# cjpurackal/nice-slam-cpp

Measured on AMD Instinct MI355X. Metric: mapping rays/sec (and ms/iter) on CoFusion room1 at 1/2/4/8 MI355X, higher is better.
Workload: dtype f32

## Files before the change

include/nsk.h:

```cpp
#ifndef NSK_H
#define NSK_H

#include <stddef.h>
#include <stdint.h>

#ifdef __cplusplus
extern "C" {
#endif

#define NSK_COARSE 0
#define NSK_MIDDLE 1
#define NSK_FINE 2
#define NSK_COLOR 3

#define NSK_GRAD_GRIDS 1u
#define NSK_GRAD_DECODERS 2u
#define NSK_GRAD_RAYS 4u

#define NSK_GROUP_DECODERS 0
#define NSK_GROUP_COARSE 1
#define NSK_GROUP_MIDDLE 2
#define NSK_GROUP_FINE 3
#define NSK_GROUP_COLOR 4
#define NSK_GROUP_CAMERA 5
// ... 13 lines not shown
int nsk_set_matmul_mode(nsk_ctx* ctx, int mode);
int nsk_set_backward_mode(nsk_ctx* ctx, int mode);

int nsk_set_sort_mode(nsk_ctx* ctx, int mode);
int nsk_set_tuning(nsk_ctx* ctx, const char* key, int value);

int nsk_set_bound(nsk_ctx* ctx, const float h_bound[6]);

int nsk_set_render_opts(nsk_ctx* ctx, int n_samples, int n_surface, int lindisp, float perturb, int occupancy,
                        uint64_t seed);

int nsk_grid_upload(nsk_ctx* ctx, int level, const float* h_czyx, int C, int Z, int Y, int X);
int nsk_grid_download(nsk_ctx* ctx, int level, float* h_czyx);
int nsk_grid_grad_download(nsk_ctx* ctx, int level, float* h_czyx);
int nsk_set_mask(nsk_ctx* ctx, int level, const uint8_t* h_mask_zyx);

int nsk_frustum_mask(nsk_ctx* ctx, int level, const float* d_depth, int H, int W, float fx, float fy, float cx, float cy,
                     const float h_c2w[16], uint8_t* h_mask_out);

int nsk_keyframe_overlap(nsk_ctx* ctx, int N, const float* d_rays_o, const float* d_rays_d, const float* d_gt_depth, int n_samples,
                         int H, int W, float fx, float fy, float cx, float cy, int K, const float* h_c2w, float* h_percent);

size_t nsk_decoder_param_count(int which);
int nsk_decoder_upload(nsk_ctx* ctx, int which, const float* h_packed, size_t n);
int nsk_decoder_download(nsk_ctx* ctx, int which, float* h_packed, size_t n);
int nsk_decoder_grad_download(nsk_ctx* ctx, int which, float* h_packed, size_t n);
int nsk_decoder_set_trainable(nsk_ctx* ctx, int which, int trainable);

int nsk_render_forward(nsk_ctx* ctx, int stage, int N, const float* d_rays_o, const float* d_rays_d,
                       const float* d_gt_depth, float gt_depth_max, float* d_rgb, float* d_depth, float* d_var,
// ... 101 lines not shown
```

nice-slam-cpp_amd/csrc/nsk.hip:

```cpp
#include "../../include/nsk.h"
#include "nsk_device.h"
#include "nsk_train.h"
#include "nsk_bf16.h"
#include "nsk_mesh.h"
#include "nsk_buf.h"

#include <dlfcn.h>
#include <cstdarg>
#include <algorithm>
#include <cmath>
#include <cstdio>
#include <cstring>
#include <memory>
#include <string>
#include <vector>

#define NSK_VERSION 100

static thread_local std::string g_err;
static int fail(const char* fmt, ...)
{
    char buf[512];
    va_list ap; va_start(ap, fmt); vsnprintf(buf, sizeof(buf), fmt, ap); va_end(ap);
    g_err = buf;
// ... 106 lines not shown
        const int v = v0 + threadIdx.x;
        const bool on = v < nvox && mask[v];
        const unsigned long long b = __builtin_amdgcn_ballot_w64(on);
        if (lane == 0) wsum[wave] = __builtin_popcountll(b);
        __syncthreads();
        int off = base;
        for (int w = 0; w < wave; ++w) off += wsum[w];
        if (on) idx[off + __builtin_popcountll(b & ((1ull << lane) - 1ull))] = v;
        __syncthreads();
        if (threadIdx.x == 0) { int t = 0; for (int w = 0; w < 16; ++w) t += wsum[w]; base += t; }
        __syncthreads();
    }
    if (threadIdx.x == 0) *count = base;
}

struct XSeg { const int* idx; int n4; float* slab; float* buf; int blk_end;
              const float* slabs; int nslabs, slab_stride; };
struct XArgs { XSeg s[10]; int n; int gather; };
__global__ __launch_bounds__(256) void k_xchg_multi(XArgs A)
{
    int r = 0;
    while (r < A.n - 1 && (int)blockIdx.x >= A.s[r].blk_end) ++r;
    const XSeg& S = A.s[r];
    const int b0 = r ? A.s[r - 1].blk_end : 0;
    if (S.slabs) {
        __shared__ f4 red[32][8];
        const int pi = threadIdx.x & 7, sg = threadIdx.x >> 3;
        const int i = (blockIdx.x - b0) * 8 + pi;
        f4 part = (f4)(0.f);
        if (i < S.n4) {
// ... 478 lines not shown
__global__ void k_gather_pixels(int n, const int* __restrict__ pi, const int* __restrict__ pj, int W, const float* __restrict__ depth,
                                const float* __restrict__ color, float* __restrict__ gd, float* __restrict__ gc)
{
    const int r = blockIdx.x * blockDim.x + threadIdx.x;
    if (r >= n) return;
    const size_t p = (size_t)pj[r] * W + pi[r];
    gd[r] = depth[p];
    if (color && gc) { gc[3 * r] = color[3 * p]; gc[3 * r + 1] = color[3 * p + 1]; gc[3 * r + 2] = color[3 * p + 2]; }
}

struct HipAlloc {
    static int alloc(void** p, size_t bytes) { return (int)hipMalloc(p, bytes); }
    static void free(void* p) { (void)hipFree(p); }
};
template <typename T> using Buf = DevBuf<T, HipAlloc>;

struct GridState {
    int C = 0, Z = 0, Y = 0, X = 0;
    size_t n = 0;
    Buf<float> v, m, s;
    Buf<uint8_t> mask;
    size_t g_off = 0;
    Buf<int> midx; int nmask = 0; bool midx_dirty = true;
};
struct DecState {
    int n = 0;
    Buf<float> p, m, s;
    Buf<float> fimg, bimg;
    Buf<int> fidx, bidx;
    Buf<int> finv, binv;
    Buf<int> inv16;
    Buf<int> invh;
    Buf<float> bimg16; Buf<int> bidx16; int bfrag16_n = 0; bool bimg16_dirty = true;
    Buf<float> fimg16; Buf<int> fidx16; int frag16_n = 0, fimg16_f = 0, tail_off = 0, tail16_off = 0, np16 = 3, cq16 = 2;
    int fimg_n = 0, bimg_n = 0;
    int trainable = 0;
// ... 39 lines not shown
    int cap_rollback[NSK_NUM_GROUPS] = {0, 0, 0, 0, 0, 0};
    int ws_flip = 0;
    struct GraphRec { bool stale = false; int flip = 0; hipGraph_t graph = nullptr; hipGraphExec_t exec = nullptr; hipGraphNode_t adam_node = nullptr; bool has_adam = false; CapAdam adam; std::vector<CapVec> vecs; };
    std::vector<GraphRec> graphs;
    bool touched[NSK_NUM_GROUPS] = {false, false, false, false, false, false};
    bool deterministic = false;
    bool roctx = false;
    int tune_fwd_occ_cost = 0, tune_no_occ_role = 0;
    int tune_fwd_fine_cost = 0, tune_fwd_color_cost = 0;
    bool median_fused_pending = false;
    int tune_no_deferred_median = 0;
    int tune_no_fused_median = 0;
    int tune_frozen_cost = 0;
    int tune_frozen_cost_rays = 0;
    int tune_frozen_mid_pct = 100;
    int tune_no_frozen_kernel = 0;
    const uint8_t* ray_mask = nullptr;
    struct DMax { const float* gt = nullptr; const uint8_t* keep = nullptr; int n = 0; } dmax;
    float* xextra = nullptr; size_t xextra_n = 0;
    int sort_mode = -1;
    bool sorted = false;
    struct Prep { bool valid = false; int stage = 0, N = 0, S = 0; const float* ro = nullptr; const float* rd = nullptr; const float* gt = nullptr;
                  float gtmax = 0.f; const uint8_t* mask = nullptr; bool sorted = false; int done = 0; RParams R; DMax dmax; } prep, req;
    int tune_no_piggyback = 0;
    int pend_w = -1, pend_nb = 0;
    int dbg_M = 0, dbg_S = 0;
    int bwd_mode = 2;
    int matmul_mode = 2;
    double last_bytes = 0, last_flops = 0; int last_samples = 0;
    struct Mesh {
// ... 125 lines not shown
    HIPCHK(hipGetDeviceProperties(&prop, device));
    if (strncmp(prop.gcnArchName, "gfx950", 6) != 0) return fail("nsk_ctx_create: device arch %s, this library is built for gfx950 only", prop.gcnArchName);
    std::unique_ptr<nsk_ctx> owner(new nsk_ctx());
    nsk_ctx* c = owner.get();
    c->device = device;
    c->num_cu = prop.multiProcessorCount;
    if (hip_stream) { c->stream = (hipStream_t)hip_stream; c->own_stream = false; }
    else { HIPCHK(hipStreamCreateWithFlags(&c->stream, hipStreamNonBlocking)); c->own_stream = true; }
    const float b[6] = {-4.5f, 3.82f, -1.5f, 2.02f, -3.0f, 2.76f};
    memcpy(c->R.bound, b, sizeof(b));
    c->R.n_samples = 32; c->R.n_surface = 16; c->R.lindisp = 0; c->R.occupancy = 0; c->R.perturb = 0.f; c->R.seed = 0;
    CHK(dev_alloc(c->d_bound, 6, "the bound"));
    HIPCHK(hipMemcpy(c->d_bound, b, sizeof(b), hipMemcpyHostToDevice));
    CHK(dev_alloc(c->scal, 16, "the scalars"));
    HIPCHK(hipMemset(c->scal, 0, 16 * sizeof(float)));
    CHK(set_lds(k_decode_fwd<0>, fwd_img_floats(0) * 4)); CHK(set_lds(k_decode_fwd<1>, fwd_img_floats(1) * 4));
    CHK(set_lds(k_decode_fwd<2>, fwd_img_floats(2) * 4)); CHK(set_lds(k_decode_fwd<3>, fwd_img_floats(3) * 4));
#define SETB(W) \
    CHK(set_lds(k_decode_bwd<W, false>, bwd_lds_bytes(W, false))); CHK(set_lds(k_decode_bwd<W, true>, bwd_lds_bytes(W, false))); \
    CHK(set_lds(k_decode_bwd_train<W, false>, bwd_lds_bytes(W, true))); CHK(set_lds(k_decode_bwd_train<W, true>, bwd_lds_bytes(W, true)));
    SETB(0) SETB(1) SETB(2) SETB(3)
#undef SETB
    CHK(set_lds(k_median_thr, 16384 * 4));
    CHK(set_lds(k_decode_fwd_multi, 160 * 1024)); CHK(set_lds(k_decode_fwd_multi_bf16<8>, 160 * 1024)); CHK(set_lds(k_decode_fwd_multi_bf16<8, 2>, 160 * 1024)); CHK(set_lds(k_decode_fwd_multi_occ<8>, 160 * 1024));
    CHK(set_lds(k_decode_bwd_multi<false>, 160 * 1024 - 256)); CHK(set_lds(k_decode_bwd_multi<true>, 160 * 1024));
    CHK(set_lds(k_decode_bwd_frozen<false>, 160 * 1024 - 256));
    CHK(set_lds(k_decode_bwd_track, 160 * 1024)); CHK(set_lds(k_decode_bwd_multi_full<false>, 160 * 1024)); CHK(set_lds(k_decode_bwd_multi_full<true>, 160 * 1024));
    CHK(set_lds(k_decode_fwd_dump<0>, 160 * 1024)); CHK(set_lds(k_decode_fwd_dump<1>, 160 * 1024)); CHK(set_lds(k_decode_fwd_dump<2>, 160 * 1024));
    *out = owner.release();
    return 0;
// ... 40 lines not shown

extern "C" int nsk_set_backward_mode(nsk_ctx* c, int mode)
{
    if (!c) return fail("null ctx");
    if (mode != 0 && mode != 2) return fail("nsk_set_backward_mode: 0 (fp32 MFMA chains) or 2 (two fp16 pieces, default)");
    c->bwd_mode = mode;
    return 0;
}

extern "C" int nsk_set_tuning(nsk_ctx* c, const char* key, int value)
{
    if (!c || !key) return fail("nsk_set_tuning: null argument");
    if (!strcmp(key, "frozen_cost")) { c->tune_frozen_cost = value; return 0; }
    if (!strcmp(key, "frozen_cost_rays")) { c->tune_frozen_cost_rays = value; return 0; }
    if (!strcmp(key, "no_frozen_kernel")) { c->tune_no_frozen_kernel = value; return 0; }
    if (!strcmp(key, "no_piggyback")) { c->tune_no_piggyback = value; return 0; }
    if (!strcmp(key, "frozen_mid_pct")) { if (value < 10 || value > 1000) return fail("nsk_set_tuning: frozen_mid_pct out of range"); c->tune_frozen_mid_pct = value; return 0; }
    if (!strcmp(key, "no_fused_median")) { c->tune_no_fused_median = value; return 0; }
    if (!strcmp(key, "no_deferred_median")) { c->tune_no_deferred_median = value; return 0; }
    if (!strcmp(key, "fwd_fine_cost")) { c->tune_fwd_fine_cost = value; return 0; }
    if (!strcmp(key, "fwd_occ_cost")) { c->tune_fwd_occ_cost = value; return 0; }
    if (!strcmp(key, "no_occ_role")) { c->tune_no_occ_role = value; return 0; }
    if (!strcmp(key, "fwd_color_cost")) { c->tune_fwd_color_cost = value; return 0; }
    if (!strcmp(key, "deterministic")) { c->deterministic = value != 0; return 0; }
    if (!strcmp(key, "roctx")) { c->roctx = value != 0; return 0; }
    if (!strcmp(key, "lattice_slab")) { if (value < 0 || value >= (1 << 26)) return fail("nsk_set_tuning: lattice_slab must be 0 (automatic) or a node count below 2^26"); c->mesh.slab = value; return 0; }
    return fail("nsk_set_tuning: unknown key '%s'", key);
}

extern "C" int nsk_set_ray_mask(nsk_ctx* c, const uint8_t* d_keep)
// ... 43 lines not shown
        c->slab_n = n;
    }
    HIPCHK(hipMemsetAsync(c->slab, 0, n * sizeof(float), c->stream));
    return 0;
}

static int grid_upload(nsk_ctx* c, GridState& G, const float* h, int C, int Z, int Y, int X)
{
    size_t nvox = (size_t)Z * Y * X, n = nvox * 32;
    bool realloc_ = n != G.n;
    if (realloc_) {
        CHK(grow_begin(c, GROW_STALE_GRAPHS));
        G = GridState();
        CHK(dev_alloc(G.v, n, "a grid level")); CHK(dev_alloc(G.m, n, "a grid level's first moment")); CHK(dev_alloc(G.s, n, "a grid level's second moment"));
    }
    if (G.Z != Z || G.Y != Y || G.X != X) { if (G.mask) { CHK(grow_begin(c, GROW_STALE_GRAPHS)); G.mask.reset(); } }
    G.C = C; G.Z = Z; G.Y = Y; G.X = X; G.n = n; G.midx_dirty = true;
    std::vector<float> t(n);
    for (int ch = 0; ch < 32; ++ch)
        for (size_t v = 0; v < nvox; ++v) t[v * 32 + ch] = h[(size_t)ch * nvox + v];
    HIPCHK(hipMemcpyAsync(G.v, t.data(), n * 4, hipMemcpyHostToDevice, c->stream));
    HIPCHK(hipMemsetAsync(G.m, 0, n * 4, c->stream));
    HIPCHK(hipMemsetAsync(G.s, 0, n * 4, c->stream));
    HIPCHK(hipStreamSynchronize(c->stream));
    if (realloc_) CHK(rebuild_slab(c));
    return 0;
}
extern "C" int nsk_grid_upload(nsk_ctx* c, int level, const float* h, int C, int Z, int Y, int X)
{
    if (!c || !h) return fail("nsk_grid_upload: null argument");
    if (!which_ok(level)) return fail("nsk_grid_upload: bad level %d", level);
// ... 28 lines not shown
extern "C" int nsk_grid_grad_download(nsk_ctx* c, int level, float* h)
{
    if (!c || !h || !which_ok(level)) return fail("nsk_grid_grad_download: bad argument");
    CHK(grid_fetch(c, level, c->slab + c->grid[level].g_off, h));
    GridState& G = c->grid[level];
    if (G.mask) {
        const size_t nvox = G.n / 32;
        std::vector<uint8_t> m(nvox);
        HIPCHK(hipMemcpy(m.data(), G.mask, nvox, hipMemcpyDeviceToHost));
        for (int ch = 0; ch < 32; ++ch)
            for (size_t v = 0; v < nvox; ++v) if (!m[v]) h[(size_t)ch * nvox + v] = 0.f;
    }
    return 0;
}

extern "C" int nsk_set_mask(nsk_ctx* c, int level, const uint8_t* h_mask)
{
    if (!c || !which_ok(level)) return fail("nsk_set_mask: bad argument");
    GridState& G = c->grid[level];
    if (!G.n) return fail("nsk_set_mask: grid level %d not uploaded", level);
    if (c->capturing) return fail("nsk_set_mask: not while a graph is being captured");
    HIPCHK(hipStreamSynchronize(c->stream));
    size_t nvox = G.n / 32;
    G.midx_dirty = true;
    invalidate_graphs(c);
    if (c->slab) HIPCHK(hipMemsetAsync(c->slab + G.g_off, 0, G.n * 4, c->stream));
    if (!h_mask) { G.mask.reset(); return 0; }
    if (!G.mask) CHK(dev_alloc(G.mask, nvox, "the voxel mask"));
    HIPCHK(hipMemcpy(G.mask, h_mask, nvox, hipMemcpyHostToDevice));
    return 0;
}

static void seg_fwd(std::vector<int>& idx, int quad0, int KQ, int Wofs, int ld, int col0, int kvalid)
{
    for (int rt = 0; rt < 2; ++rt) for (int q = 0; q < KQ; ++q) for (int lane = 0; lane < 64; ++lane) for (int i = 0; i < 4; ++i) {
        int o = 16 * rt + (lane & 15), k = 16 * q + 4 * (lane >> 4) + i;
        idx[((size_t)(quad0 + rt * KQ + q) * 64 + lane) * 4 + i] = k < kvalid ? Wofs + o * ld + col0 + k : -1;
    }
}
static void seg_bwd(std::vector<int>& idx, int quad0, int RT, int Wofs, int ld, int col0, int rvalid)
{
    const int KQ = 2;
    for (int rt = 0; rt < RT; ++rt) for (int q = 0; q < KQ; ++q) for (int lane = 0; lane < 64; ++lane) for (int i = 0; i < 4; ++i) {
        int r = 16 * rt + (lane & 15), k = 16 * q + 4 * (lane >> 4) + i;
// ... 884 lines not shown
    }
    return T.ntri[case_index];
}

static int flush_pending(nsk_ctx* c)
{
    if (c->pend_w < 0) return 0;
    const int w = c->pend_w, np = c->dec[w].n, n4 = (np + 3) & ~3;
    ProfScope ps(c, "dec_grad_reduce");
    k_dec_grad_reduce<<<dim3((np + 255) / 256, 8), 256, 0, c->stream>>>(np, n4, c->pend_nb, c->ws.dec_slabs, c->slab + c->dec[w].g_off);
    HIPCHK(hipGetLastError());
    c->pend_w = -1;
    return 0;
}

static int backward_core(nsk_ctx* c, int stage, int N, int S, const float* ro, const float* rd, unsigned flags, float* g_ro, float* g_rd,
                         float* d_loss = nullptr, const float* dyn_resid = nullptr)
{
    const bool rays = (flags & NSK_GRAD_RAYS) != 0;
    const bool grids = (flags & NSK_GRAD_GRIDS) != 0;
    const int M = N * S;
    CHK(flush_pending(c));
    MultiArgs MA;
    memset(&MA, 0, sizeof(MA));
    int n = 0, cost[3], train_role = -1; size_t lds = 0;
    for (int q = 2; q >= 0; --q) {
        int w = STAGE_DEC[stage][q];
        if (w < 0) continue;
        bool train = (flags & NSK_GRAD_DECODERS) && c->dec[w].trainable;
        if (!train && !grids && !rays) continue;
// ... 2 lines not shown
        A.grid = grid_dev(c, w, grids);
        A.masks = c->ws.masks[w];
        A.g_raw = c->ws.g_raw;
        A.g_rays_o = g_ro; A.g_rays_d = g_rd;
        A.dyn_resid = dyn_resid; A.dyn_n = N;
        A.g_dec = train ? c->ws.dec_slabs : c->slab + c->dec[w].g_off;
        A.flags = flags & 0xffu;
        if (w != 0 && (!train || w != 2)) CHK(ensure_bimg16(c, w));
        if (train && w != 2) {
            if (c->ws.hsave_M[w] != M) return fail("backward of trainable decoder %d: its forward must run with the decoder already trainable (block outputs not saved)", w);
            A.hsave = c->ws.hsave[w];
        }
        MA.which[n] = w; MA.train[n] = train ? 1 : 0;
        const int frozen_cost = rays ? (c->tune_frozen_cost_rays > 0 ? c->tune_frozen_cost_rays : 330) : (c->tune_frozen_cost > 0 ? c->tune_frozen_cost : 205);
        cost[n] = train ? 1000 : (w == 1 ? frozen_cost * c->tune_frozen_mid_pct / 100 : frozen_cost);
        lds = std::max(lds, bwd_lds_bytes(w, train));
        if (train) train_role = (train_role == -1 && w != 2) ? n : -2;
        if (train) c->touched[NSK_GROUP_DECODERS] = true;
        if (grids) c->touched[NSK_GROUP_COARSE + w] = true;
        ++n;
    }
    if (dyn_resid && (train_role != -1 || !rays || c->deterministic || c->bwd_mode == 0 || n == 0 || N > NSK_MEDIAN_FUSED_MAX))
        return fail("backward_core: the deferred median mask needs the Tracker's launch (frozen decoders, ray gradients)");
    const int separate = c->deterministic ? 1 : 0;
    if ((n == 0 || train_role == -2 || separate) && d_loss) { ProfScope ps(c, "loss_sum"); k_sum<<<1, 1024, 0, c->stream>>>(N, c->ws.ray_loss, d_loss); }
    if (n == 0) return 0;
    if (train_role == -2 || separate) {
        for (int r = 0; r < n; ++r)
            CHK(launch_decode_bwd(c, MA.which[r], M, S, ro, rd, MA.train[r] != 0, rays, flags, g_ro, g_rd));
        return 0;
// ... 285 lines not shown
extern "C" int nsk_frustum_mask(nsk_ctx* c, int level, const float* d_depth, int H, int W, float fx, float fy, float cx, float cy,
                                const float h_c2w[16], uint8_t* h_mask_out)
{
    if (!c || !which_ok(level) || !d_depth || !h_c2w) return fail("nsk_frustum_mask: bad argument");
    GridState& G = c->grid[level];
    if (!G.n) return fail("nsk_frustum_mask: grid level %d not uploaded", level);
    HIPCHK(hipSetDevice(c->device));
    const size_t nvox = G.n / 32;
    G.midx_dirty = true;
    if (c->capturing) return fail("nsk_frustum_mask: not while a graph is being captured");
    bool live = false;
    for (auto& R : c->graphs) live = live || !R.stale;
    if (live) { HIPCHK(hipStreamSynchronize(c->stream)); invalidate_graphs(c); }
    if (c->slab) HIPCHK(hipMemsetAsync(c->slab + G.g_off, 0, G.n * 4, c->stream));
    CHK(grow(c, G.mask, nvox, "the voxel mask", 0));
    if (level == NSK_COARSE) {
        HIPCHK(hipMemsetAsync(G.mask, 1, nvox, c->stream));
    } else {
        CHK(grow(c, c->fr_tmp, nvox * 9 + 16, "the frustum scratch", 0));
        float* dep = reinterpret_cast<float*>(c->fr_tmp.get()); float* zz = dep + nvox;
        uint8_t* inimg = reinterpret_cast<uint8_t*>(zz + nvox);
        unsigned int* dmax = reinterpret_cast<unsigned int*>(c->scal + 4);
        FrustumArgs A;
        memcpy(A.bound, c->R.bound, sizeof(A.bound));
        invert4(h_c2w, A.w2c);
        A.cam[0] = h_c2w[3]; A.cam[1] = h_c2w[7]; A.cam[2] = h_c2w[11];
        A.Z = G.Z; A.Y = G.Y; A.X = G.X; A.H = H; A.W = W; A.fx = fx; A.fy = fy; A.cx = cx; A.cy = cy;
        HIPCHK(hipMemsetAsync(dmax, 0, 4, c->stream));
        int blocks = (int)((nvox + 255) / 256);
        k_frustum_pass1<<<blocks, 256, 0, c->stream>>>(A, d_depth, dep, zz, inimg, dmax);
        k_frustum_pass2<<<blocks, 256, 0, c->stream>>>(A, dep, zz, inimg, dmax, G.mask);
        HIPCHK(hipGetLastError());
    }
    if (h_mask_out) {
        HIPCHK(hipMemcpyAsync(h_mask_out, G.mask, nvox, hipMemcpyDeviceToHost, c->stream));
        HIPCHK(hipStreamSynchronize(c->stream));
    }
    return 0;
}

extern "C" int nsk_keyframe_overlap(nsk_ctx* c, int N, const float* d_ro, const float* d_rd, const float* d_gt_depth, int n_samples,
                                    int H, int W, float fx, float fy, float cx, float cy, int K, const float* h_c2w, float* h_percent)
{
    if (!c || !d_ro || !d_rd || !d_gt_depth || !h_c2w || !h_percent) return fail("nsk_keyframe_overlap: null argument");
    if (N <= 0 || n_samples <= 0 || K < 0) return fail("nsk_keyframe_overlap: bad sizes");
    if (K == 0) return 0;
    HIPCHK(hipSetDevice(c->device));
    std::vector<float> w2c((size_t)K * 16);
// ... 537 lines not shown
```

nice-slam-cpp_amd/csrc/nsk_device.h:

```cpp
#pragma once
#include <hip/hip_runtime.h>
#include <stdint.h>
#include "nsk_layout.h"

typedef float f4 __attribute__((ext_vector_type(4)));

struct RParams {
    float bound[6];
    int n_samples, n_surface, lindisp, occupancy;
    float perturb;
    unsigned long long seed;
};

struct GridD {
    const float* v;
    float* g;
    const uint8_t* mask;
    int Z, Y, X;
};

#define NSK_INF __builtin_huge_valf()

__device__ __forceinline__ f4 mfma4(float a, float b, f4 c) { return __builtin_amdgcn_mfma_f32_16x16x4f32(a, b, c, 0, 0, 0); }
__device__ __forceinline__ void lds_fence() { asm volatile("s_waitcnt lgkmcnt(0)" ::: "memory"); }
// ... 667 lines not shown
    const f4* img;
    const void* img16;
    const f4* bimg;
    const void* bimg16;
    int img_f4;
    float* out;
    unsigned long long* masks;
    f4* hsave;
    const float* g_raw;
    float* g_rays_o; float* g_rays_d;
    float* g_dec;
    unsigned flags;
    float* dump;
    const float* dyn_resid;
    int dyn_n;
};

template <typename T>
__device__ __forceinline__ T ld32(const void* base, unsigned byte_off) { return *reinterpret_cast<const T*>(reinterpret_cast<const char*>(base) + byte_off); }
__device__ __forceinline__ int ray_of(const DecArgs& A, int mm) { return A.S_magic ? (int)__umulhi((unsigned)mm, A.S_magic) : mm; }
struct __attribute__((packed, aligned(4))) Ray3 { float x, y, z; };
__device__ __forceinline__ void sample_point(const DecArgs& A, int mm, float& px, float& py, float& pz, float& zz, int& n)
{
    if (A.pts) { px = A.pts[3 * mm]; py = A.pts[3 * mm + 1]; pz = A.pts[3 * mm + 2]; zz = 0.f; n = 0; return; }
    n = ray_of(A, mm);
    zz = A.z[mm];
    const Ray3 o = *reinterpret_cast<const Ray3*>(A.rays_o + 3 * n), d = *reinterpret_cast<const Ray3*>(A.rays_d + 3 * n);
    px = add_rn(o.x, mul_rn(d.x, zz));
    py = add_rn(o.y, mul_rn(d.y, zz));
    pz = add_rn(o.z, mul_rn(d.z, zz));
// ... 485 lines not shown
template <int K> struct ImgRegs { f4 v[K]; };
template <int NT, int K>
__device__ __forceinline__ void image_issue(ImgRegs<K>& R, const f4* __restrict__ src, int n4)
{
#pragma unroll
    for (int u = 0; u < K; ++u) { const int i = u * NT + (int)threadIdx.x; R.v[u] = i < n4 ? src[i] : (f4)(0.f); }
}
template <int NT, int K>
__device__ __forceinline__ void image_commit(f4* __restrict__ dst, const ImgRegs<K>& R, const f4* __restrict__ src, int n4)
{
#pragma unroll
    for (int u = 0; u < K; ++u) { const int i = u * NT + (int)threadIdx.x; if (i < n4) dst[i] = R.v[u]; }
    if (n4 > K * NT) copy_image_to_lds<NT>(dst + K * NT, src + K * NT, n4 - K * NT);
}

template <int WHICH, bool RAYS, int NW = 8, bool FULL = false, bool DYN = false>
__device__ __forceinline__ void decode_bwd_body(const DecArgs& A, int bid, int nb)
{
    static_assert(!DYN || RAYS, "the deferred median mask belongs to the Tracker's ray-gradient launch");
    constexpr bool XYZ = WHICH != 0;
    constexpr int OD = WHICH == 3 ? 4 : 1;
    constexpr bool NEED_E = XYZ && RAYS;
    constexpr bool B16 = XYZ && !FULL;
    constexpr int IMG_F = B16 ? MlpBwdImgH::TOTAL_F : (XYZ ? MlpBwdImg::TOTAL : CoarseBwdImg::TOTAL);
    extern __shared__ __attribute__((aligned(16))) f4 smem[];
    const int wave = __builtin_amdgcn_readfirstlane(threadIdx.x >> 6), lane = threadIdx.x & 63, j = lane & 15, g = lane >> 4;
    float* smf = reinterpret_cast<float*>(smem);
    float* scratch = smf + IMG_F + wave * 960;
    float* dyn_rs = smf + IMG_F + NW * 960;
    float dyn_thr = 0.f;
    const f4* img_src = B16 ? reinterpret_cast<const f4*>(A.bimg16) : A.bimg;
    constexpr int IMG_K = (IMG_F / 4 + 64 * NW - 1) / (64 * NW) < 8 ? (IMG_F / 4 + 64 * NW - 1) / (64 * NW) : 8;
    ImgRegs<IMG_K> img_regs;
    const f4* bimg = smem;
// ... 25 lines not shown
            float rv[PER];
#pragma unroll
            for (int e = 0; e < PER; ++e) { const int i = (int)threadIdx.x + e * 64 * NW; rv[e] = i < A.dyn_n ? A.dyn_resid[i] : NSK_INF; }
            image_commit<64 * NW>(smem, img_regs, img_src, IMG_F / 4);
#pragma unroll
            for (int e = 0; e < PER; ++e) { const int i = (int)threadIdx.x + e * 64 * NW; if (i < NSK_MEDIAN_FUSED_MAX) dyn_rs[i] = rv[e]; }
            __syncthreads();
            dyn_thr = lower_median_x10<64 * NW, NSK_MEDIAN_FUSED_MAX>(dyn_rs, (A.dyn_n + 3) & ~3, reinterpret_cast<int*>(dyn_rs + NSK_MEDIAN_FUSED_MAX));
        } else {
            image_commit<64 * NW>(smem, img_regs, img_src, IMG_F / 4);
            __syncthreads();
        }
    }
    int mm_next = slot_sample(A, slot_of(tile_of(1, wg, nw, tsh)));
    const bool det = (A.flags & 0x8000u) != 0;
    for (int k = 0; k < kmax; ++k) {
        const int task = tile_of(k, wg, nw, tsh);
        if (task >= ntasks && !det) break;
        asm volatile("" ::: "memory");
        const bool valid = task * 16 + j < A.M;
        const int mm = nx.mm;
        float px, py, pz;
        sample_finish(A, nx.r, px, py, pz);
        const float zz = A.pts ? 0.f : nx.r.z;
        const int n = A.pts ? 0 : ray_of(A, mm);
        Tri T;
        tri_setup(A.grid, A.bound, px, py, pz, T);
        float gout[OD];
        {
            f4 gr = nx.gr;
            if (!valid) gr = (f4)(0.f);
            if constexpr (DYN) { if (!(dyn_rs[n] < dyn_thr)) gr = (f4)(0.f); }
            if constexpr (OD == 4) { gout[0] = gr[0]; gout[1] = gr[1]; gout[2] = gr[2]; gout[3] = 0.f; }
            else gout[0] = gr[3];
        }
        float unscale = 1.f;
        if constexpr (B16) unscale = chain_scale<OD>(gout);
        const unsigned long long mask = nx.mask;
        stage(tile_of(k + 1, wg, nw, tsh), mm_next, nx);
        mm_next = slot_sample(A, slot_of(tile_of(k + 2, wg, nw, tsh)));
        f4 xcos[6];
        if constexpr (NEED_E) { f4 e[6]; embed<true>(Bm, g, px, py, pz, e, xcos); }
        f4 gh[2];
#pragma unroll
        for (int r = 0; r < 2; ++r)
#pragma unroll
            for (int i = 0; i < 4; ++i) {
                float s = 0.f;
#pragma unroll
                for (int o = 0; o < OD; ++o) s += Wo[32 * o + 16 * r + 4 * g + i] * gout[o];
                gh[r][i] = s;
            }
        f4 gc[2] = {(f4)(0.f), (f4)(0.f)}, gcL[2] = {(f4)(0.f), (f4)(0.f)};
        f4 ge[6];
#pragma unroll
// ... 85 lines not shown
#pragma unroll
                    for (int k = 0; k < 3; ++k) {
                        atomicAdd(A.g_rays_o + 3 * n + k, gp[k]);
                        atomicAdd(A.g_rays_d + 3 * n + k, gp[k] * zz);
                    }
                }
                if (det) asm volatile("s_waitcnt vmcnt(0)" ::: "memory");
            }
        }
        if ((A.flags & 1u) && A.grid.g) {
            if (det) {
                for (int w = 0; w < NW; ++w) { if (wave == w) { scatter_tile(A.grid, T, gc, lane, valid, scratch); asm volatile("s_waitcnt vmcnt(0)" ::: "memory"); } __syncthreads(); }
            } else scatter_tile(A.grid, T, gc, lane, valid, scratch);
        }
    }
}

template <int WHICH, bool RAYS>
__global__ __launch_bounds__(512) void k_decode_bwd(DecArgs A) { decode_bwd_body<WHICH, RAYS>(A, blockIdx.x, gridDim.x); }

#define NSK_FROZEN_NW 16
template <bool RAYS>
__global__ __launch_bounds__(64 * NSK_FROZEN_NW) void k_decode_bwd_frozen(MultiArgs MA)
{
    if (MA.sum_n > 0 && blockIdx.x == gridDim.x - 1) { block_sum(MA.sum_src, MA.sum_n, MA.sum_dst); return; }
    if ((int)blockIdx.x >= MA.wg_end[MA.n - 1]) { sort_scan_body<NSK_FROZEN_NW / 4>(MA.scan, (int)blockIdx.x - MA.wg_end[MA.n - 1]); return; }
    int r = 0;
    while (r < MA.n - 1 && (int)blockIdx.x >= MA.wg_end[r]) ++r;
    const int b0 = r == 0 ? 0 : MA.wg_end[r - 1];
    const int bid = blockIdx.x - b0, nb = MA.wg_end[r] - b0;
    switch (MA.which[r]) {
    case 0: decode_bwd_body<0, RAYS, NSK_FROZEN_NW>(MA.a[r], bid, nb); break;
    case 1: decode_bwd_body<1, RAYS, NSK_FROZEN_NW>(MA.a[r], bid, nb); break;
    case 2: decode_bwd_body<2, RAYS, NSK_FROZEN_NW>(MA.a[r], bid, nb); break;
    default: decode_bwd_body<3, RAYS, NSK_FROZEN_NW>(MA.a[r], bid, nb); break;
    }
}

#define NSK_DYN_LDS_BYTES (NSK_MEDIAN_FUSED_MAX * 4 + 3 * 8 * 4)
__global__ __launch_bounds__(512) void k_decode_bwd_track(MultiArgs MA)
{
    if (blockIdx.x == gridDim.x - 1) {
        extern __shared__ __attribute__((aligned(16))) f4 smem[];
        float* rs = reinterpret_cast<float*>(smem);
        const DecArgs& A = MA.a[0];
// ... 34 lines not shown
```

nice-slam-cpp_amd/csrc/nsk_train.h:

```cpp
#pragma once
#include "nsk_device.h"
#include <type_traits>
#include <utility>

#define PN_RB 272
#define PN_GROWS 32
#define PN_EROWS(CQ) (PN_GROWS + 16 * (CQ))
#define PN_ROWS(CQ) (PN_EROWS(CQ) + 96)
#define PN_MOFF(CQ) (PN_ROWS(CQ) * PN_RB)
#define PN_FLOATS(CQ) (2 * PN_MOFF(CQ) / 4)

struct TrainPhase {
    int RT, NC, rowsum;
    int slot0, nslots;
    int w_base, ld, col0;
    int rows, cols_total;
    int b_base;
};

template <int WHICH>
struct TrainPlan {
    static constexpr bool XYZ = WHICH != 0;
    static constexpr int CQ = WHICH == 2 ? 4 : 2;
    static constexpr int OD = WHICH == 3 ? 4 : 1;
// ... 1051 lines not shown
template <int WHICH, bool RAYS>
__global__ __launch_bounds__(512) void k_decode_bwd_train(DecArgs A) { decode_bwd_train_any<WHICH, RAYS>(A, blockIdx.x, gridDim.x); }

template <bool RAYS>
__global__ __launch_bounds__(512) void k_decode_bwd_multi(MultiArgs MA)
{
    if (MA.sum_n > 0 && blockIdx.x == gridDim.x - 1) { block_sum(MA.sum_src, MA.sum_n, MA.sum_dst); return; }
    if constexpr (!RAYS) {
        if ((int)blockIdx.x >= MA.wg_end[MA.n - 1]) { sort_scan_body<2>(MA.scan, (int)blockIdx.x - MA.wg_end[MA.n - 1]); return; }
    }
    int r = 0;
    while (r < MA.n - 1 && (int)blockIdx.x >= MA.wg_end[r]) ++r;
    const int b0 = r == 0 ? 0 : MA.wg_end[r - 1];
    const int bid = blockIdx.x - b0, nb = MA.wg_end[r] - b0;
    const int sel = MA.which[r] * 2 + (MA.train[r] ? 1 : 0);
    switch (sel) {
    case 0: decode_bwd_body<0, RAYS>(MA.a[r], bid, nb); break;
    case 1: decode_bwd_train_any<0, RAYS>(MA.a[r], bid, nb); break;
    case 2: decode_bwd_body<1, RAYS>(MA.a[r], bid, nb); break;
    case 3: decode_bwd_train_any<1, RAYS>(MA.a[r], bid, nb); break;
    case 4: decode_bwd_body<2, RAYS>(MA.a[r], bid, nb); break;
    case 5: break;
    case 6: decode_bwd_body<3, RAYS>(MA.a[r], bid, nb); break;
    default: decode_bwd_train_any<3, RAYS>(MA.a[r], bid, nb); break;
    }
}

template <bool RAYS>
__global__ __launch_bounds__(512) void k_decode_bwd_multi_full(MultiArgs MA)
{
// ... 18 lines not shown
```

nice-slam-cpp_amd/nsk.py:

```python
import ctypes as C
import os
import subprocess

_HERE = os.path.dirname(os.path.abspath(__file__))
_LIB_PATH = os.environ.get("NSK_LIB", os.path.join(_HERE, "csrc", "libnsk.so"))

STAGES = {"coarse": 0, "middle": 1, "fine": 2, "color": 3}
LEVELS = ("coarse", "middle", "fine", "color")
GRAD_GRIDS, GRAD_DECODERS, GRAD_RAYS = 1, 2, 4
GROUP_DECODERS, GROUP_COARSE, GROUP_MIDDLE, GROUP_FINE, GROUP_COLOR, GROUP_CAMERA = range(6)

SYMBOLS = (
    "nsk_last_error", "nsk_version", "nsk_ctx_create", "nsk_ctx_destroy", "nsk_sync", "nsk_stream", "nsk_set_bound",
    "nsk_set_render_opts", "nsk_set_matmul_mode", "nsk_set_sort_mode", "nsk_set_tuning", "nsk_set_ray_mask", "nsk_grid_upload", "nsk_grid_download", "nsk_grid_grad_download", "nsk_set_mask", "nsk_frustum_mask", "nsk_keyframe_overlap", "nsk_sample_pixels", "nsk_gather_pixels", "nsk_rays_from_camera", "nsk_pose_step",
    "nsk_decoder_param_count", "nsk_decoder_upload", "nsk_decoder_download", "nsk_decoder_grad_download",
    "nsk_decoder_set_trainable", "nsk_render_forward", "nsk_eval_points", "nsk_raw2outputs", "nsk_render_backward", "nsk_map_step",
    "nsk_track_step", "nsk_loss_map", "nsk_loss_track", "nsk_rays_from_pixels", "nsk_rays_backward",
    "nsk_camera_from_tensor", "nsk_camera_backward", "nsk_inside_filter", "nsk_adam_vector", "nsk_adam_step",
    "nsk_adam_reset", "nsk_graph_begin", "nsk_graph_end", "nsk_graph_launch", "nsk_graph_destroy", "nsk_zero_grads", "nsk_prepare_rays", "nsk_map_prepare", "nsk_grad_slab", "nsk_grad_pack", "nsk_grad_unpack", "nsk_allreduce_grads", "nsk_last_call_stats",
    "nsk_profile_begin", "nsk_profile_end", "nsk_debug_relu_bits", "nsk_debug_preact", "nsk_debug_fetch",
    "nsk_pose_step_multi", "nsk_set_depth_max_batch", "nsk_grad_extra", "nsk_set_backward_mode",
    "nsk_eval_lattice", "nsk_mesh_extract", "nsk_mesh_buffers", "nsk_mesh_download", "nsk_mesh_table",
)


class NskError(RuntimeError):
    pass


# ... 139 lines not shown

    def grid_download(self, level, grad=False):
        import numpy as np
        out = np.zeros(self._gshape[_stage(level)], np.float32)
        f = lib().nsk_grid_grad_download if grad else lib().nsk_grid_download
        _chk(f(self.h, _stage(level), out.ctypes.data_as(C.c_void_p)))
        return out

    def set_mask(self, level, mask):
        import numpy as np
        if mask is None:
            _chk(lib().nsk_set_mask(self.h, _stage(level), None))
            return
        m = np.ascontiguousarray(np.asarray(mask).astype(np.uint8))
        _chk(lib().nsk_set_mask(self.h, _stage(level), m.ctypes.data_as(C.c_void_p)))

    @_ordered
    def frustum_mask(self, level, depth_img, intr, c2w):
        import numpy as np
        H, W = depth_img.shape
        Cc, Z, Y, X = self._gshape[_stage(level)]
        m = np.ascontiguousarray(np.asarray(c2w, dtype=np.float32).reshape(4, 4))
        out = np.zeros(Z * Y * X, np.uint8)
        fx, fy, cx, cy = intr
        _chk(lib().nsk_frustum_mask(self.h, _stage(level), _ptr(depth_img), H, W, C.c_float(fx), C.c_float(fy), C.c_float(cx),
                                    C.c_float(cy), m.ctypes.data_as(C.c_void_p), out.ctypes.data_as(C.c_void_p)))
        return out.reshape(Z, Y, X).astype(bool)

    @_ordered
    def sample_pixels(self, seed, n, H0, H1, W0, W1):
# ... 383 lines not shown
```

Measured before the change: 14.41 million.

## Skip backward tiles whose voxel cells lie entirely outside the grid mask

Builds a per-cell liveness map from the voxel mask (a cell is live if any of its 8 corner voxels is masked) and adds a SKIP variant of the frozen-decoder backward kernel. Tiles where no lane touches a live cell skip the decoder backward and scatter work. Each launch reports its live-tile count into pinned host memory, and the work-group cost balancer reads that to reweight the frozen roles. The gradients of masked-out voxels are presumably discarded later anyway, so this only removes wasted work. It adds a kernel launch whenever a mask is set, per-launch atomics and a fence, and cost estimates that lag one launch behind.

```diff
diff --git a/include/nsk.h b/include/nsk.h
--- a/include/nsk.h
+++ b/include/nsk.h
@@ -51,6 +51,7 @@
 int nsk_grid_download(nsk_ctx* ctx, int level, float* h_czyx);
 int nsk_grid_grad_download(nsk_ctx* ctx, int level, float* h_czyx);
 int nsk_set_mask(nsk_ctx* ctx, int level, const uint8_t* h_mask_zyx);
+int nsk_dead_skip_stats(nsk_ctx* ctx, int which, int* tiles_computed, int* tiles);
 
 int nsk_frustum_mask(nsk_ctx* ctx, int level, const float* d_depth, int H, int W, float fx, float fy, float cx, float cy,
                      const float h_c2w[16], uint8_t* h_mask_out);
diff --git a/nice-slam-cpp_amd/csrc/nsk.hip b/nice-slam-cpp_amd/csrc/nsk.hip
--- a/nice-slam-cpp_amd/csrc/nsk.hip
+++ b/nice-slam-cpp_amd/csrc/nsk.hip
@@ -144,6 +144,20 @@
     if (threadIdx.x == 0) *count = base;
 }
 
+__global__ __launch_bounds__(256) void k_cell_live(int Z, int Y, int X, const uint8_t* __restrict__ mask, uint8_t* __restrict__ live)
+{
+    const int v = blockIdx.x * 256 + threadIdx.x;
+    if (v >= Z * Y * X) return;
+    const int ix = v % X, iy = (v / X) % Y, iz = v / (X * Y);
+    unsigned m = 0;
+#pragma unroll
+    for (int c = 0; c < 8; ++c) {
+        const int jx = min(ix + (c & 1), X - 1), jy = min(iy + ((c >> 1) & 1), Y - 1), jz = min(iz + (c >> 2), Z - 1);
+        m |= mask[(jz * Y + jy) * X + jx];
+    }
+    live[v] = m ? 1 : 0;
+}
+
 struct XSeg { const int* idx; int n4; float* slab; float* buf; int blk_end;
               const float* slabs; int nslabs, slab_stride; };
 struct XArgs { XSeg s[10]; int n; int gather; };
@@ -652,12 +666,17 @@
     static void free(void* p) { (void)hipFree(p); }
 };
 template <typename T> using Buf = DevBuf<T, HipAlloc>;
+struct HipHostAlloc {
+    static int alloc(void** p, size_t bytes) { return (int)hipHostMalloc(p, bytes, hipHostMallocMapped); }
+    static void free(void* p) { (void)hipHostFree(p); }
+};
 
 struct GridState {
     int C = 0, Z = 0, Y = 0, X = 0;
     size_t n = 0;
     Buf<float> v, m, s;
     Buf<uint8_t> mask;
+    Buf<uint8_t> live;
     size_t g_off = 0;
     Buf<int> midx; int nmask = 0; bool midx_dirty = true;
 };
@@ -727,6 +746,10 @@
     int tune_frozen_cost = 0;
     int tune_frozen_cost_rays = 0;
     int tune_frozen_mid_pct = 100;
+    Buf<unsigned> live_cnt;
+    DevBuf<unsigned long long, HipHostAlloc> live_host;
+    bool live_skipped[4] = {false, false, false, false}; int live_tiles[4] = {0, 0, 0, 0};
+    int tune_no_dead_skip = 0;
     int tune_no_frozen_kernel = 0;
     const uint8_t* ray_mask = nullptr;
     struct DMax { const float* gt = nullptr; const uint8_t* keep = nullptr; int n = 0; } dmax;
@@ -882,6 +905,10 @@
     HIPCHK(hipMemcpy(c->d_bound, b, sizeof(b), hipMemcpyHostToDevice));
     CHK(dev_alloc(c->scal, 16, "the scalars"));
     HIPCHK(hipMemset(c->scal, 0, 16 * sizeof(float)));
+    CHK(dev_alloc(c->live_cnt, 8, "the live-tile counters"));
+    HIPCHK(hipMemset(c->live_cnt, 0, 8 * sizeof(unsigned)));
+    if (c->live_host.alloc(4) != 0) { (void)hipGetLastError(); return fail("nsk_ctx_create: cannot allocate the pinned live-tile words"); }
+    memset(c->live_host.get(), 0, 4 * sizeof(unsigned long long));
     CHK(set_lds(k_decode_fwd<0>, fwd_img_floats(0) * 4)); CHK(set_lds(k_decode_fwd<1>, fwd_img_floats(1) * 4));
     CHK(set_lds(k_decode_fwd<2>, fwd_img_floats(2) * 4)); CHK(set_lds(k_decode_fwd<3>, fwd_img_floats(3) * 4));
 #define SETB(W) \
@@ -952,6 +979,7 @@
     if (!strcmp(key, "frozen_cost")) { c->tune_frozen_cost = value; return 0; }
     if (!strcmp(key, "frozen_cost_rays")) { c->tune_frozen_cost_rays = value; return 0; }
     if (!strcmp(key, "no_frozen_kernel")) { c->tune_no_frozen_kernel = value; return 0; }
+    if (!strcmp(key, "no_dead_skip")) { c->tune_no_dead_skip = value; return 0; }
     if (!strcmp(key, "no_piggyback")) { c->tune_no_piggyback = value; return 0; }
     if (!strcmp(key, "frozen_mid_pct")) { if (value < 10 || value > 1000) return fail("nsk_set_tuning: frozen_mid_pct out of range"); c->tune_frozen_mid_pct = value; return 0; }
     if (!strcmp(key, "no_fused_median")) { c->tune_no_fused_median = value; return 0; }
@@ -1025,7 +1053,7 @@
         G = GridState();
         CHK(dev_alloc(G.v, n, "a grid level")); CHK(dev_alloc(G.m, n, "a grid level's first moment")); CHK(dev_alloc(G.s, n, "a grid level's second moment"));
     }
-    if (G.Z != Z || G.Y != Y || G.X != X) { if (G.mask) { CHK(grow_begin(c, GROW_STALE_GRAPHS)); G.mask.reset(); } }
+    if (G.Z != Z || G.Y != Y || G.X != X) { if (G.mask) { CHK(grow_begin(c, GROW_STALE_GRAPHS)); reset_all(G.mask, G.live); } }
     G.C = C; G.Z = Z; G.Y = Y; G.X = X; G.n = n; G.midx_dirty = true;
     std::vector<float> t(n);
     for (int ch = 0; ch < 32; ++ch)
@@ -1084,6 +1112,29 @@
     return 0;
 }
 
+static int build_cell_live(nsk_ctx* c, GridState& G)
+{
+    const int nvox = (int)(G.n / 32);
+    k_cell_live<<<(nvox + 255) / 256, 256, 0, c->stream>>>(G.Z, G.Y, G.X, G.mask, G.live);
+    HIPCHK(hipGetLastError());
+    return 0;
+}
+
+extern "C" int nsk_dead_skip_stats(nsk_ctx* c, int which, int* tiles_computed, int* tiles)
+{
+    if (!c || !which_ok(which) || !tiles_computed || !tiles) return fail("nsk_dead_skip_stats: bad argument");
+    HIPCHK(hipSetDevice(c->device));
+    HIPCHK(hipStreamSynchronize(c->stream));
+    *tiles = c->live_tiles[which];
+    *tiles_computed = c->live_tiles[which];
+    if (c->live_skipped[which]) {
+        const unsigned long long v = *const_cast<volatile unsigned long long*>(c->live_host.get() + which);
+        if ((int)(v >> 32) != c->live_tiles[which]) return fail("nsk_dead_skip_stats: the last launch of decoder %d has not reported", which);
+        *tiles_computed = (int)(v & 0xffffffffu);
+    }
+    return 0;
+}
+
 extern "C" int nsk_set_mask(nsk_ctx* c, int level, const uint8_t* h_mask)
 {
     if (!c || !which_ok(level)) return fail("nsk_set_mask: bad argument");
@@ -1095,9 +1146,14 @@
     G.midx_dirty = true;
     invalidate_graphs(c);
     if (c->slab) HIPCHK(hipMemsetAsync(c->slab + G.g_off, 0, G.n * 4, c->stream));
-    if (!h_mask) { G.mask.reset(); return 0; }
-    if (!G.mask) CHK(dev_alloc(G.mask, nvox, "the voxel mask"));
+    c->live_host.get()[level] = 0;
+    if (!h_mask) { reset_all(G.mask, G.live); return 0; }
+    if (!G.mask) {
+        const int r = [&]() -> int { CHK(dev_alloc(G.mask, nvox, "the voxel mask")); CHK(dev_alloc(G.live, nvox, "the mask's cell map")); return 0; }();
+        if (r != 0) { reset_all(G.mask, G.live); return r; }
+    }
     HIPCHK(hipMemcpy(G.mask, h_mask, nvox, hipMemcpyHostToDevice));
+    CHK(build_cell_live(c, G));
     return 0;
 }
 
@@ -2012,6 +2068,7 @@
     return 0;
 }
 
+#define NSK_DEAD_TILE_PCT 15
 static int backward_core(nsk_ctx* c, int stage, int N, int S, const float* ro, const float* rd, unsigned flags, float* g_ro, float* g_rd,
                          float* d_loss = nullptr, const float* dyn_resid = nullptr)
 {
@@ -2044,6 +2101,15 @@
         MA.which[n] = w; MA.train[n] = train ? 1 : 0;
         const int frozen_cost = rays ? (c->tune_frozen_cost_rays > 0 ? c->tune_frozen_cost_rays : 330) : (c->tune_frozen_cost > 0 ? c->tune_frozen_cost : 205);
         cost[n] = train ? 1000 : (w == 1 ? frozen_cost * c->tune_frozen_mid_pct / 100 : frozen_cost);
+        const GridState& G = c->grid[w];
+        if (!train) { c->live_skipped[w] = false; c->live_tiles[w] = (M + 15) / 16; }
+        if (!train && grids && !rays && !c->deterministic && c->bwd_mode != 0 && !c->tune_no_dead_skip && G.mask && G.live) {
+            A.live = G.live; A.live_cnt = c->live_cnt + 2 * w; A.live_host = c->live_host.get() + w;
+            c->live_skipped[w] = true;
+            const unsigned long long v = *const_cast<volatile unsigned long long*>(c->live_host.get() + w);
+            const long tot = (long)(v >> 32), live = (long)(v & 0xffffffffu);
+            if (tot > 0 && live <= tot) cost[n] = std::max(1, (int)((long)cost[n] * (live * 100 + (tot - live) * NSK_DEAD_TILE_PCT) / (tot * 100)));
+        }
         lds = std::max(lds, bwd_lds_bytes(w, train));
         if (train) train_role = (train_role == -1 && w != 2) ? n : -2;
         if (train) c->touched[NSK_GROUP_DECODERS] = true;
@@ -2359,6 +2425,8 @@
     if (live) { HIPCHK(hipStreamSynchronize(c->stream)); invalidate_graphs(c); }
     if (c->slab) HIPCHK(hipMemsetAsync(c->slab + G.g_off, 0, G.n * 4, c->stream));
     CHK(grow(c, G.mask, nvox, "the voxel mask", 0));
+    { const int r = grow(c, G.live, nvox, "the mask's cell map", 0); if (r != 0) { reset_all(G.mask, G.live); return r; } }
+    c->live_host.get()[level] = 0;
     if (level == NSK_COARSE) {
         HIPCHK(hipMemsetAsync(G.mask, 1, nvox, c->stream));
     } else {
@@ -2377,6 +2445,7 @@
         k_frustum_pass2<<<blocks, 256, 0, c->stream>>>(A, dep, zz, inimg, dmax, G.mask);
         HIPCHK(hipGetLastError());
     }
+    CHK(build_cell_live(c, G));
     if (h_mask_out) {
         HIPCHK(hipMemcpyAsync(h_mask_out, G.mask, nvox, hipMemcpyDeviceToHost, c->stream));
         HIPCHK(hipStreamSynchronize(c->stream));
diff --git a/nice-slam-cpp_amd/csrc/nsk_device.h b/nice-slam-cpp_amd/csrc/nsk_device.h
--- a/nice-slam-cpp_amd/csrc/nsk_device.h
+++ b/nice-slam-cpp_amd/csrc/nsk_device.h
@@ -705,6 +705,9 @@
     float* dump;
     const float* dyn_resid;
     int dyn_n;
+    const uint8_t* live;
+    unsigned* live_cnt;
+    unsigned long long* live_host;
 };
 
 template <typename T>
@@ -1220,10 +1223,11 @@
     if (n4 > K * NT) copy_image_to_lds<NT>(dst + K * NT, src + K * NT, n4 - K * NT);
 }
 
-template <int WHICH, bool RAYS, int NW = 8, bool FULL = false, bool DYN = false>
+template <int WHICH, bool RAYS, int NW = 8, bool FULL = false, bool DYN = false, bool SKIP = false>
 __device__ __forceinline__ void decode_bwd_body(const DecArgs& A, int bid, int nb)
 {
     static_assert(!DYN || RAYS, "the deferred median mask belongs to the Tracker's ray-gradient launch");
+    static_assert(!SKIP || (!RAYS && !FULL), "ray gradients need every tile");
     constexpr bool XYZ = WHICH != 0;
     constexpr int OD = WHICH == 3 ? 4 : 1;
     constexpr bool NEED_E = XYZ && RAYS;
@@ -1279,6 +1283,7 @@
     }
     int mm_next = slot_sample(A, slot_of(tile_of(1, wg, nw, tsh)));
     const bool det = (A.flags & 0x8000u) != 0;
+    [[maybe_unused]] unsigned n_live = 0;
     for (int k = 0; k < kmax; ++k) {
         const int task = tile_of(k, wg, nw, tsh);
         if (task >= ntasks && !det) break;
@@ -1300,10 +1305,17 @@
             else gout[0] = gr[3];
         }
         float unscale = 1.f;
-        if constexpr (B16) unscale = chain_scale<OD>(gout);
+        [[maybe_unused]] unsigned cell_live = 0;
+        if constexpr (SKIP) cell_live = valid ? (unsigned)ld32<uint8_t>(A.live, (unsigned)T.vox[0]) : 0u;
+        else if constexpr (B16) unscale = chain_scale<OD>(gout);
         const unsigned long long mask = nx.mask;
         stage(tile_of(k + 1, wg, nw, tsh), mm_next, nx);
         mm_next = slot_sample(A, slot_of(tile_of(k + 2, wg, nw, tsh)));
+        if constexpr (SKIP) {
+            if (__builtin_amdgcn_ballot_w64(cell_live != 0u) == 0ull) continue;
+            ++n_live;
+            if constexpr (B16) unscale = chain_scale<OD>(gout);
+        }
         f4 xcos[6];
         if constexpr (NEED_E) { f4 e[6]; embed<true>(Bm, g, px, py, pz, e, xcos); }
         f4 gh[2];
@@ -1419,6 +1431,18 @@
             } else scatter_tile(A.grid, T, gc, lane, valid, scratch);
         }
     }
+    if constexpr (SKIP) {
+        if (lane == 0) {
+            atomicAdd(A.live_cnt, n_live);
+            __threadfence();
+            if (atomicAdd(A.live_cnt + 1, 1u) == (unsigned)nw - 1u) {
+                __threadfence();
+                const unsigned total = atomicExch(A.live_cnt, 0u);
+                atomicExch(A.live_cnt + 1, 0u);
+                __hip_atomic_store(A.live_host, ((unsigned long long)(unsigned)ntasks << 32) | total, __ATOMIC_RELEASE, __HIP_MEMORY_SCOPE_SYSTEM);
+            }
+        }
+    }
 }
 
 template <int WHICH, bool RAYS>
@@ -1434,6 +1458,17 @@
     while (r < MA.n - 1 && (int)blockIdx.x >= MA.wg_end[r]) ++r;
     const int b0 = r == 0 ? 0 : MA.wg_end[r - 1];
     const int bid = blockIdx.x - b0, nb = MA.wg_end[r] - b0;
+    if constexpr (!RAYS) {
+        if (MA.a[r].live) {
+            switch (MA.which[r]) {
+            case 0: decode_bwd_body<0, false, NSK_FROZEN_NW, false, false, true>(MA.a[r], bid, nb); break;
+            case 1: decode_bwd_body<1, false, NSK_FROZEN_NW, false, false, true>(MA.a[r], bid, nb); break;
+            case 2: decode_bwd_body<2, false, NSK_FROZEN_NW, false, false, true>(MA.a[r], bid, nb); break;
+            default: decode_bwd_body<3, false, NSK_FROZEN_NW, false, false, true>(MA.a[r], bid, nb); break;
+            }
+            return;
+        }
+    }
     switch (MA.which[r]) {
     case 0: decode_bwd_body<0, RAYS, NSK_FROZEN_NW>(MA.a[r], bid, nb); break;
     case 1: decode_bwd_body<1, RAYS, NSK_FROZEN_NW>(MA.a[r], bid, nb); break;
diff --git a/nice-slam-cpp_amd/csrc/nsk_train.h b/nice-slam-cpp_amd/csrc/nsk_train.h
--- a/nice-slam-cpp_amd/csrc/nsk_train.h
+++ b/nice-slam-cpp_amd/csrc/nsk_train.h
@@ -1089,6 +1089,17 @@
     const int b0 = r == 0 ? 0 : MA.wg_end[r - 1];
     const int bid = blockIdx.x - b0, nb = MA.wg_end[r] - b0;
     const int sel = MA.which[r] * 2 + (MA.train[r] ? 1 : 0);
+    if constexpr (!RAYS) {
+        if (MA.a[r].live) {
+            switch (sel) {
+            case 0: decode_bwd_body<0, false, 8, false, false, true>(MA.a[r], bid, nb); break;
+            case 2: decode_bwd_body<1, false, 8, false, false, true>(MA.a[r], bid, nb); break;
+            case 4: decode_bwd_body<2, false, 8, false, false, true>(MA.a[r], bid, nb); break;
+            default: decode_bwd_body<3, false, 8, false, false, true>(MA.a[r], bid, nb); break;
+            }
+            return;
+        }
+    }
     switch (sel) {
     case 0: decode_bwd_body<0, RAYS>(MA.a[r], bid, nb); break;
     case 1: decode_bwd_train_any<0, RAYS>(MA.a[r], bid, nb); break;
diff --git a/nice-slam-cpp_amd/nsk.py b/nice-slam-cpp_amd/nsk.py
--- a/nice-slam-cpp_amd/nsk.py
+++ b/nice-slam-cpp_amd/nsk.py
@@ -12,7 +12,7 @@
 
 SYMBOLS = (
     "nsk_last_error", "nsk_version", "nsk_ctx_create", "nsk_ctx_destroy", "nsk_sync", "nsk_stream", "nsk_set_bound",
-    "nsk_set_render_opts", "nsk_set_matmul_mode", "nsk_set_sort_mode", "nsk_set_tuning", "nsk_set_ray_mask", "nsk_grid_upload", "nsk_grid_download", "nsk_grid_grad_download", "nsk_set_mask", "nsk_frustum_mask", "nsk_keyframe_overlap", "nsk_sample_pixels", "nsk_gather_pixels", "nsk_rays_from_camera", "nsk_pose_step",
+    "nsk_set_render_opts", "nsk_set_matmul_mode", "nsk_set_sort_mode", "nsk_set_tuning", "nsk_set_ray_mask", "nsk_grid_upload", "nsk_grid_download", "nsk_grid_grad_download", "nsk_set_mask", "nsk_dead_skip_stats", "nsk_frustum_mask", "nsk_keyframe_overlap", "nsk_sample_pixels", "nsk_gather_pixels", "nsk_rays_from_camera", "nsk_pose_step",
     "nsk_decoder_param_count", "nsk_decoder_upload", "nsk_decoder_download", "nsk_decoder_grad_download",
     "nsk_decoder_set_trainable", "nsk_render_forward", "nsk_eval_points", "nsk_raw2outputs", "nsk_render_backward", "nsk_map_step",
     "nsk_track_step", "nsk_loss_map", "nsk_loss_track", "nsk_rays_from_pixels", "nsk_rays_backward",
@@ -182,6 +182,11 @@
             return
         m = np.ascontiguousarray(np.asarray(mask).astype(np.uint8))
         _chk(lib().nsk_set_mask(self.h, _stage(level), m.ctypes.data_as(C.c_void_p)))
+
+    def dead_skip_stats(self, which):
+        live, tiles = C.c_int(0), C.c_int(0)
+        _chk(lib().nsk_dead_skip_stats(self.h, _stage(which), C.byref(live), C.byref(tiles)))
+        return live.value, tiles.value
 
     @_ordered
     def frustum_mask(self, level, depth_img, intr, c2w):
```

Result: slower. 13.53 million (-6.1%).
